# superlinear-ai/raglite

Measured on AMD Instinct MI355X. Metric: queries/sec, MaxSim 32x1M d=1024 exact top-100, higher is better.
Workload: dtype f32 in / f32 scores: candidate chunks found with the fp16 hi halves of corpus and queries (1 x v_mfma_f32_16x16x32_f16 per multiply, f32 accumulate, rigorous error bound), their scores by v_mfma_f32_16x16x4_f32 (exact f32 products); full-precision fallback: 3 x v_mfma_f32_16x16x32_f16 on hi+lo pairs

## Files before the change

raglite_amd/csrc/api.hip:

```cpp
#include <cmath>
#include <cstdlib>
#include <cstring>
#include <limits>
#include <memory>
#include <mutex>
#include <utility>
#include <vector>

#include "handles.h"

namespace rl {

static thread_local std::string g_last_error;
void set_error(const std::string& msg) { g_last_error = msg; }
int fail(int code, const std::string& msg) {
    g_last_error = msg;
    return code;
}

namespace {

int scan_mode(int metric) {
    switch (metric) {
        case RL_COSINE: return SCAN_COSINE;
// ... 106 lines not shown
bool image_fits(const rl_index* idx, const rl::Pool& pool, size_t need) {
    if (pool.cap >= need) return true;
    size_t free_b = 0, total_b = 0;
    if (hipMemGetInfo(&free_b, &total_b) != hipSuccess) { (void)hipGetLastError(); return true; }
    return free_b + pool.cap >= need + image_headroom(idx);
}
int64_t image_cap_rows(const rl_index* idx) { return std::max<int64_t>(idx->n_rows, idx->owns_E() ? idx->cap_rows : idx->n_rows); }

int refresh_ends(rl_index* idx, hipStream_t s) {
    if (idx->ends_rows == idx->n_rows && idx->ends.p) return RL_OK;
    RL_TRY(idx->ends.reserve(rl::chunk_ends_words(image_cap_rows(idx)) * sizeof(uint32_t)));
    RL_TRY(rl::launch_chunk_ends(idx->row_to_chunk, idx->n_rows, idx->ends.as<uint32_t>(), s));
    idx->ends_rows = idx->n_rows;
    return RL_OK;
}

int fold_row_norms(rl_index* idx, int64_t from, hipStream_t s) {
    rl::NormStats& ns = idx->norm_stats;
    RL_TRY(idx->d_norms.reserve(16));
    float w[4] = {ns.max_row_norm, ns.max_lo_norm, ns.max_lo_ratio, ns.min_row_norm};
    RL_HIP(hipMemcpyAsync(idx->d_norms, w, sizeof(w), hipMemcpyHostToDevice, s));
    const size_t at = (size_t)from * idx->dim;
    RL_TRY(idx->E16 ? rl::launch_max_row_norm16(idx->E16 + at, idx->n_rows - from, idx->dim, idx->d_norms, s)
                    : rl::launch_max_row_norm(idx->E + at, idx->n_rows - from, idx->dim, idx->split_scale, idx->d_norms, s));
    RL_HIP(hipMemcpyAsync(w, idx->d_norms, sizeof(w), hipMemcpyDeviceToHost, s));
    RL_HIP(hipStreamSynchronize(s));
    ns.max_row_norm = w[0];
    ns.max_lo_norm = w[1];
    ns.max_lo_ratio = w[2];
    ns.min_row_norm = w[3];
// ... 24 lines not shown
bool image_wanted(const rl_index* idx, uint32_t bit) {
    const int32_t d = idx->dim;
    if (!(image_need(idx) & bit) || idx->n_rows <= 0) return false;
    if (bit == IMG_PLANES) return idx->opt.on(RL_OPT_KEEP_IMAGE) && (idx->E16 || idx->E) && image_scale(idx) > 0.f && d % 32 == 0 && d >= 32;
    const bool hi = idx->opt.on(RL_OPT_KEEP_HI) && !idx->E16 && idx->E && idx->split_scale > 0.f && big_corpus(idx);
    if (bit == IMG_HI_IMAGE) return hi && hi_dim_ok(d);
    return hi && idx->opt.on(RL_OPT_KEEP_HI_PLANE) && stream16_dim_ok(d) &&
           (idx->metric == RL_COSINE || idx->metric == RL_DOT || idx->metric == RL_L2);
}

int refresh_image(rl_index* idx, uint32_t bit, hipStream_t s) {
    rl::Image& im = image_record(idx, bit);
    const bool tiled = bit != IMG_HI_PLANE;
    const int64_t n = idx->n_rows;
    const int32_t d = idx->dim;
    if (bit == IMG_PLANES) idx->ends_rows = -1;
    if (!image_wanted(idx, bit)) {
        im.drop();
        return RL_OK;
    }
    const float scale = image_scale(idx);
    const int64_t cap = image_cap_rows(idx);
    const size_t need = tiled ? rl::planes_bytes(cap, d, bit == IMG_HI_IMAGE || idx->E16) : (size_t)cap * d * sizeof(uint16_t);
    int64_t first = im.scale == scale ? (tiled ? im.rows & ~int64_t(15) : im.rows) : 0;
    if (im.buf.cap < need) first = 0;
    if (!image_fits(idx, im.buf, need) || im.buf.reserve(need) != RL_OK) {
        (void)hipGetLastError();
        idx->no_room |= bit;
        im.drop();
        return RL_OK;
    }
// ... 1449 lines not shown
    return (size_t)n * k * 3 + (size_t)n * 3 + 16 + (size_t)n * 2048 * 2 + 2 + 2 * pivot_scratch_words(std::min<int32_t>(n, 2));
}
int hi_batch_approx(rl_index* idx, const float* d_q, int32_t nq, int32_t n_queries, int32_t n_gemm, int32_t k, float* sc, int64_t ld, HiBatch& hb,
                    hipStream_t s, bool flag_zeroed = false) {
    hb.one_product = idx->opt.v[RL_OPT_HI_PRODUCTS] == 1;
    hb.exact_kth = idx->opt.on(RL_OPT_EXACT_KTH_THRESHOLD);
    RL_TRY(idx->hibuf.reserve(hi_batch_words(n_gemm, k) * 4));
    hi_batch_layout(idx, n_gemm, k, hb);
    const int32_t cap = hb.cap;
    hb.m_abs = idx->norm_stats.max_lo_norm + sum_eps(idx->dim) * idx->norm_stats.max_row_norm;
    hb.q_unscale = reinterpret_cast<const float*>(idx->qplanes.as<char>() + (size_t)n_queries * idx->dim * 128);
    hb.qsum = hb.q_unscale + 2 * (size_t)n_queries;
    if (!flag_zeroed) RL_HIP(hipMemsetAsync(hb.flag, 0, 16 * sizeof(uint32_t), s));
    (void)cap;
    const bool pp = hb.one_product && idx->dim >= 256 && idx->opt.on(RL_OPT_PP_PASS);
    if (pp)
        RL_TRY(launch_maxsim_pp(approx_image(idx), idx->n_rows, idx->dim, idx->qplanes.p, n_queries, 0, n_gemm, nq, idx->row_to_chunk,
                                idx->offsets, idx->ends.as<uint32_t>(), sc, ld, idx->n_cu, s, approx_scale(idx), nullptr,
                                (int)idx->opt.v[RL_OPT_PP_SCHEDULE], (int)idx->opt.v[RL_OPT_PP_XCD_PASSES]));
    for (int32_t b = 0; !pp && b < n_gemm; b += GEMM_PASS_QUERIES) {
        const int32_t n_q = std::min<int32_t>(GEMM_PASS_QUERIES, n_gemm - b);
        RL_TRY(launch_maxsim_gemm(approx_image(idx), idx->n_rows, idx->dim, idx->qplanes.p, n_queries, b, n_q, nq, idx->row_to_chunk,
                                  idx->offsets, idx->ends.as<uint32_t>(), sc + (int64_t)b * ld, ld, idx->n_cu, s, approx_scale(idx), true,
                                  nullptr, hb.one_product));
    }
    RL_TRY(mask_chunk_scores(idx, sc, n_gemm, ld, hb.filter, s));
    int st_pv = RL_ERR_UNSUPPORTED;
    if (n_gemm < 16 && idx->n_chunks > (int64_t)262144 && idx->opt.on(RL_OPT_HI_PIVOT))
        st_pv = launch_topk_pivot(sc, n_gemm, idx->n_chunks, ld, k, idx->ws, hb.ts, hb.ti, s);
    if (st_pv != RL_OK && st_pv != RL_ERR_UNSUPPORTED) return st_pv;
    if (st_pv == RL_ERR_UNSUPPORTED) RL_TRY(launch_topk(sc, n_gemm, idx->n_chunks, ld, k, idx->ws, hb.ts, hb.ti, s));
    return RL_OK;
}
int hi_batch_fallback(rl_index* idx, const float* d_q, int32_t nq, int32_t n_queries, int32_t n_gemm, int32_t k, float* sc, int64_t ld,
// ... 327 lines not shown
    if (idx->has_empty_chunk || idx->n_chunks == 0)
        return fail(RL_ERR_UNSUPPORTED, "rl_maxsim_approx_scores: the approximate pass needs an index without empty chunks");
    RL_TRY(demand_images(idx, approx_image_bit(idx), s));
    if (!approx_image_valid(idx) || nq > 32 || (kernel == 0 && idx->dim < 256))
        return fail(RL_ERR_UNSUPPORTED, "rl_maxsim_approx_scores: this index keeps no HI image (or nq > 32 / dim < 256)");
    Staging st(mem, s);
    const float* d_q; float* d_o; float* d_b = nullptr;
    const size_t q_elems = (size_t)nq * idx->dim;
    const int64_t ld = idx->n_chunks;
    RL_TRY(st.in(query_vecs, (size_t)n_queries * q_elems, &d_q));
    RL_TRY(st.out(out_scores, (size_t)n_queries * ld, &d_o));
    RL_TRY(st.out(out_bound, (size_t)n_queries, &d_b));
    RL_TRY(idx->qplanes.reserve(query_planes_bytes(idx->dim, n_queries)));
    RL_TRY(launch_query_planes(d_q, idx->dim, nq, (int64_t)q_elems, n_queries, idx->qplanes.p, s));
    const int32_t per = kernel == 0 ? n_queries : GEMM_PASS_QUERIES;
    for (int32_t b = 0; b < n_queries; b += per) {
        const int32_t n_q = std::min<int32_t>(per, n_queries - b);
        if (kernel == 0)
            RL_TRY(launch_maxsim_pp(approx_image(idx), idx->n_rows, idx->dim, idx->qplanes.p, n_queries, b, n_q, nq, idx->row_to_chunk, idx->offsets,
                                    idx->ends.as<uint32_t>(), d_o + (int64_t)b * ld, ld, idx->n_cu, s, approx_scale(idx), nullptr,
                                    (int)idx->opt.v[RL_OPT_PP_SCHEDULE], (int)idx->opt.v[RL_OPT_PP_XCD_PASSES]));
        else
            RL_TRY(launch_maxsim_gemm(approx_image(idx), idx->n_rows, idx->dim, idx->qplanes.p, n_queries, b, n_q, nq, idx->row_to_chunk, idx->offsets,
                                      idx->ends.as<uint32_t>(), d_o + (int64_t)b * ld, ld, idx->n_cu, s, approx_scale(idx), true, nullptr, true));
    }
    if (d_b) {
        const float m_abs = idx->norm_stats.max_lo_norm + sum_eps(idx->dim) * idx->norm_stats.max_row_norm;
        const float* q_unscale = reinterpret_cast<const float*>(idx->qplanes.as<char>() + (size_t)n_queries * idx->dim * 128);
        RL_TRY(idx->hibuf.reserve((size_t)n_queries * 4 * sizeof(float) + 64));
        float* top = idx->hibuf.as<float>();
        float* thr = top + n_queries;
        uint32_t* cnt = reinterpret_cast<uint32_t*>(thr + n_queries);
        uint32_t* flag = cnt + n_queries;
        RL_HIP(hipMemsetAsync(top, 0, (size_t)n_queries * sizeof(float), s));
        RL_HIP(hipMemsetAsync(flag, 0, 16 * sizeof(uint32_t), s));
// ... 195 lines not shown
    RL_HIP(hipEventCreate(&e0));
    RL_HIP(hipEventCreate(&e1));
    int st = RL_OK;
    if (kind == 2) {
        st = pairs_prepare(idx, q_dev, nq / 2, (int64_t)(nq / 2) * idx->dim, 2, s);
        if (st != RL_OK) { (void)hipEventDestroy(e0); (void)hipEventDestroy(e1); return st == RL_ERR_UNSUPPORTED ? fail(st, "rl_time_kernel: the pair kernel does not apply to this index / shape") : st; }
    }
    if (kind == 3 || kind == 5 || kind == 6) {
        st = gemm_prepare(idx, q_dev, nq / GEMM_PASS_QUERIES, (int64_t)(nq / GEMM_PASS_QUERIES) * idx->dim, GEMM_PASS_QUERIES, s, true);
        if (st == RL_OK && !image_valid(idx)) st = RL_ERR_UNSUPPORTED;
        if (st != RL_OK) { (void)hipEventDestroy(e0); (void)hipEventDestroy(e1); return st == RL_ERR_UNSUPPORTED ? fail(st, "rl_time_kernel: the eight-query kernel does not apply to this index / shape") : st; }
    }
    if (kind == 7) {
        st = pp_vec >= 1 && pp_vec * pp_n == nq ? gemm_prepare(idx, q_dev, pp_vec, (int64_t)pp_vec * idx->dim, pp_n, s) : RL_ERR_UNSUPPORTED;
        if (st == RL_OK && !(approx_image_valid(idx) && idx->dim >= 256)) st = RL_ERR_UNSUPPORTED;
        if (st != RL_OK) { (void)hipEventDestroy(e0); (void)hipEventDestroy(e1); return st == RL_ERR_UNSUPPORTED ? fail(st, "rl_time_kernel: the sixteen-query kernel does not apply to this index / shape") : st; }
    }
    if (kind == 4 || kind == 10) {
        st = demand_images(idx, IMG_HI_PLANE, s);
        if (st != RL_OK) { (void)hipEventDestroy(e0); (void)hipEventDestroy(e1); return st; }
    }
    RL_HIP(hipEventRecord(e0, s));
    for (int i = 0; i < iters && st == RL_OK; ++i) {
        if (kind == 7) st = launch_maxsim_pp(approx_image(idx), idx->n_rows, idx->dim, idx->qplanes.p, pp_n, 0, pp_n,
                                             pp_vec, idx->row_to_chunk, idx->offsets, idx->ends.as<uint32_t>(), idx->scores.as<float>(), ldc,
                                             idx->n_cu, s, approx_scale(idx), nullptr, (int)idx->opt.v[RL_OPT_PP_SCHEDULE], (int)idx->opt.v[RL_OPT_PP_XCD_PASSES]);
        else if (kind == 3) st = gemm_pass(idx, nq / GEMM_PASS_QUERIES, GEMM_PASS_QUERIES, 0, GEMM_PASS_QUERIES, idx->scores.as<float>(), ldc, s);
        else if (kind == 8) {
            const auto& r = idx->replay;
            if (hipMemsetAsync(r.cnt, 0, (size_t)r.B * sizeof(uint32_t), s) != hipSuccess) st = RL_ERR_HIP;
            else if (r.pp && r.round1_tiles > 0) {
                CandArgs ca1 = r.ca;
                ca1.tau = r.thr1;
                st = launch_pp_rows_pass(idx->hi_image.buf.p, idx->n_rows, idx->dim, r.B, r.qs, idx->norm, r.mode, &ca1, idx->pp_work.p, r.log_cap, idx->n_cu, s,
                                         idx->split_scale, 0, r.round1_tiles, false, r.row_test);
                if (st == RL_OK)
                    st = launch_pp_rows_pass(idx->hi_image.buf.p, idx->n_rows, idx->dim, r.B, r.qs, idx->norm, r.mode, &r.ca, idx->pp_work.p, r.log_cap, idx->n_cu, s,
                                             idx->split_scale, r.round1_tiles, -1, true, r.row_test);
            }
            else if (r.pp) st = launch_pp_rows_pass(idx->hi_image.buf.p, idx->n_rows, idx->dim, r.B, r.qs, idx->norm, r.mode, &r.ca, idx->pp_work.p, r.log_cap,
// ... 39 lines not shown
```

raglite_amd/csrc/common.h:

```cpp
#pragma once
#include <hip/hip_runtime.h>
#include <stdint.h>

#include <algorithm>
#include <cstdlib>
#include <string>

#include "raglite_hip.h"

namespace rl {

void set_error(const std::string& msg);
int fail(int code, const std::string& msg);

#define RL_HIP(expr)                                                                         \
    do {                                                                                     \
        hipError_t _e = (expr);                                                              \
        if (_e != hipSuccess)                                                                \
            return ::rl::fail(_e == hipErrorOutOfMemory ? RL_ERR_NOMEM : RL_ERR_HIP,         \
                              std::string(#expr) + ": " + hipGetErrorString(_e));            \
    } while (0)

#define RL_TRY(expr)              \
    do {                          \
// ... 382 lines not shown
                          float* out, int64_t out_stride, int n_cu, hipStream_t s, float split_scale);
size_t planes_bytes(int64_t rows, int32_t dim, bool half = false);
int launch_presplit_rows(const float* E, int64_t first_row, int64_t n_rows, int32_t dim, float scale, void* planes, hipStream_t s);
int launch_preformat_rows16(const uint16_t* E, int64_t first_row, int64_t n_rows, int32_t dim, void* planes, hipStream_t s);
int launch_presplit_hi_rows(const float* E, int64_t first_row, int64_t n_rows, int32_t dim, float scale, void* planes, hipStream_t s);
size_t chunk_ends_words(int64_t rows);
int launch_chunk_ends(const int32_t* row_to_chunk, int64_t n_rows, uint32_t* ends, hipStream_t s);
size_t query_planes_bytes(int32_t dim, int32_t n_queries);
int launch_query_planes(const float* Q, int32_t dim, int32_t nq, int64_t q_stride, int32_t n_queries, void* buf, hipStream_t s,
                        uint32_t* zero_words = nullptr, int n_zero = 0);
int launch_maxsim_gemm(const void* planes, int64_t n_rows, int32_t dim, const void* qbuf, int32_t n_queries, int32_t first,
                       int32_t n_q, int32_t nq, const int32_t* row_to_chunk, const int64_t* chunk_offsets, const uint32_t* ends_bits,
                       float* out, int64_t out_stride, int n_cu, hipStream_t s, float split_scale, bool half = false,
                       const uint32_t* run_if = nullptr, bool hi_only = false, bool all_passes = false);
constexpr int32_t PP_PASS_QUERIES = 16;
int launch_maxsim_pp(const void* image, int64_t n_rows, int32_t dim, const void* qbuf, int32_t n_queries, int32_t first, int32_t n_q,
                     int32_t nq, const int32_t* row_to_chunk, const int64_t* chunk_offsets, const uint32_t* ends_bits, float* out,
                     int64_t out_stride, int n_cu, hipStream_t s, float split_scale, const uint32_t* run_if, int schedule, int xcd_passes);
constexpr int32_t MFMA_RATE_ITERS = 1000;
int launch_mfma_f16_rate(float* out, int n_cu, int32_t iters, hipStream_t s, double* flops);
size_t score_planes_scratch_floats(int32_t nb, int32_t dim);
int launch_score_planes(const void* planes, int64_t n_rows, int32_t dim, const float* Q, int32_t nb, float* scores, int64_t ld,
                        const float* row_norm, const float* row_sumsq, float* scratch, int mode, int n_cu, hipStream_t s, float split_scale,
                        bool half = false);
struct CandArgs { const float* tau; int32_t tau_stride; float* scores; int32_t* ids; uint32_t* cnt; uint32_t* overflow; int32_t cap; };
int launch_score_planes_queries(const float* Q, int32_t nb, int32_t dim, float* scratch, int mode, hipStream_t s, uint32_t* zero_word = nullptr);
size_t pp_rows_scratch_bytes(int64_t n_rows, int32_t nb, int n_cu, int32_t expected_per_query, int32_t* log_cap_out);
int launch_pp_rows_pass(const void* image, int64_t n_rows, int32_t dim, int32_t nb, float* scratch, const float* row_norm, int mode,
                        const CandArgs* cand, void* work, int32_t log_cap, int n_cu, hipStream_t s, float split_scale, int64_t tile_begin = 0,
                        int64_t tile_count = -1, bool norms_ready = false,
                        bool row_norm_test = false);
int launch_pp_rows_sample(const void* image, int64_t n_rows, int32_t dim, int32_t nb, float* scratch, const float* row_norm, int mode, float* S,
// ... 33 lines not shown
```

raglite_amd/csrc/handles.h:

```cpp
#pragma once
#include <limits>
#include <memory>
#include <mutex>
#include <vector>

#include "device_mem.h"

namespace rl {

inline int filters_mem(int mem) { return (mem & RL_MEM_FILTERS_DEVICE) ? RL_MEM_DEVICE : mem; }
inline int args_mem(int mem) { return mem & ~RL_MEM_FILTERS_DEVICE; }

constexpr size_t SCORE_BATCH_BYTES = size_t(8) << 30;

struct Options {
    int64_t v[RL_OPT_PP_XCD_PASSES + 1];
    Options() {
        for (auto& x : v) x = 0;
        v[RL_OPT_HI_SEARCH] = v[RL_OPT_HI_MAXSIM] = v[RL_OPT_HI_PRODUCTS] = v[RL_OPT_PP_PASS] = v[RL_OPT_FUSED_TOPK] = v[RL_OPT_FUSED_HI] = 1;
        v[RL_OPT_FUSED_PP] = v[RL_OPT_GEMM_PASS] = v[RL_OPT_QUERY_PAIRS] = v[RL_OPT_PLANES_GEMM] = v[RL_OPT_KEEP_IMAGE] = v[RL_OPT_KEEP_HI] = 1;
        v[RL_OPT_EXACT_KTH_THRESHOLD] = v[RL_OPT_FUSED_TWO_ROUNDS] = v[RL_OPT_KEEP_HI_PLANE] = v[RL_OPT_F16_EXACT] = v[RL_OPT_LAZY_IMAGES] = v[RL_OPT_FUSED_PP_SAMPLE] = v[RL_OPT_LIST_SELECT] = v[RL_OPT_HI_FEW] = 1;
        v[RL_OPT_TOPK_BLOCK] = v[RL_OPT_PAIRS_PACKED] = 2;
        v[RL_OPT_HI_PIVOT] = 1;
        v[RL_OPT_PP_SCHEDULE] = 1;
// ... 97 lines not shown
    rl::Pool ends, qplanes;
    rl::Pool q32;
    rl::Pool cand;
    rl::Pool fused;
    rl::Pool pp_work;
    rl::Pool rankbuf;
    rl::Pool hybrid;
    rl::Pool rerank;
    rl::Image hiplane;
    rl::Pool hibuf;
    rl::Image hi_image;
    rl::NormStats norm_stats;
    rl::DevArray<uint32_t> d_norms;
    rl::LastStream last_stream;
    int64_t ends_rows = -1;
    int32_t rank_B = 0;
    int32_t mb_B = 0, mb_nq = 0, mb_k = 0;
    uint64_t scratch_epoch = 0, mb_epoch = 0;
    rl::Pool rank_q;
    struct FilterRecord { int kind = 0; int32_t n = 0, cap = 0; const uint32_t* cnt = nullptr; const uint32_t* flag = nullptr; } filt;
    rl::Options opt;
    uint32_t demanded = 0;
    uint32_t no_room = 0;
    uint64_t no_room_retry_epoch = 0;
    std::unique_ptr<uint32_t, hipError_t (*)(void*)> h_fell_back{nullptr, hipHostFree};
    uint32_t* d_fell_back = nullptr;
    struct FusedReplay {
        bool valid = false, pp = false, row_test = false; int32_t B = 0, log_cap = 0; int mode = 0; float* qs = nullptr; rl::CandArgs ca{}; uint32_t* cnt = nullptr;
        const float* thr1 = nullptr; int64_t round1_tiles = 0;
        const void* pools[3] = {nullptr, nullptr, nullptr};
// ... 42 lines not shown
```

raglite_amd/csrc/maxsim_pp.hip:

```cpp
#include <cstdio>
#include <cstdlib>
#include <utility>

#include "common.h"
#include "pp_schedule.h"

namespace rl {

typedef float f32x4 __attribute__((ext_vector_type(4)));
typedef _Float16 h16x8 __attribute__((ext_vector_type(8)));

namespace {
constexpr int PP_RT = 128;
constexpr int PP_NBLK = PP_RT / 16;
constexpr int PP_QPP = 16;
constexpr int PP_DC = 8;
constexpr int PP_LC = 6;
constexpr int PP_CSLOT = PP_NBLK * 1024;
constexpr int PP_STAGE = 1536;
constexpr int PP_LDS = PP_DC * PP_CSLOT + 16 * PP_STAGE * 4;

__device__ __forceinline__ int64_t pp_uniform_i64(int64_t v) {
    const uint32_t lo = __builtin_amdgcn_readfirstlane((uint32_t)(uint64_t)v);
    const uint32_t hi = __builtin_amdgcn_readfirstlane((uint32_t)((uint64_t)v >> 32));
// ... 43 lines not shown
    const float* q_unscale;
    const float* q_sumsq;
    const float* row_norm;
    const float* blk_minmax;
    int32_t B, QT, metric;
    float* cand_scores; int32_t* cand_ids; uint32_t* cand_cnt; uint32_t* overflow; int32_t cap;
    uint2* log; int32_t log_cap;
    int32_t tile_begin, tile_count;
    float* S; int64_t ld_s; int32_t stride;
    int32_t xcd_passes, dma_hint;
};

template <int DBG, int MODE, bool ROWNORM>
__global__ __launch_bounds__(512, 2) void maxsim_pp_kernel(const char* __restrict__ planes, int64_t n_rows, int32_t nslab,
                                                           const char* __restrict__ qfrag, const float* __restrict__ qmeta, int32_t n_q,
                                                           const int32_t* __restrict__ row_to_chunk, const int64_t* __restrict__ chunk_offsets,
                                                           const uint32_t* __restrict__ ends_bits, float* __restrict__ out, int64_t out_stride,
                                                           float inv_e_scale, const uint32_t* __restrict__ run_if, PpRows rs) {
    constexpr bool ROWS = MODE == 2, SCORES = MODE == 1, GROUPS = ROWS || SCORES;
    __shared__ __attribute__((aligned(16))) char smem[PP_LDS];
    if (run_if && __builtin_amdgcn_readfirstlane((int)*run_if) == 0) return;
    const int lane = threadIdx.x & 63;
    const int wv = wave_id();
    int64_t G = gridDim.x, b = blockIdx.x;
    int qt = (int)blockIdx.y;
    if constexpr (!GROUPS) {
        const int32_t passes = (n_q + PP_QPP - 1) / PP_QPP;
        const PpSlot m = gridDim.y > 1 ? pp_schedule((int32_t)blockIdx.x, (int32_t)blockIdx.y, (int32_t)gridDim.x, (int32_t)gridDim.y, passes)
                                       : pp_schedule_affine((int32_t)blockIdx.x, (int32_t)gridDim.x, passes, rs.xcd_passes);
        G = __builtin_amdgcn_readfirstlane(m.ranges);
        b = __builtin_amdgcn_readfirstlane(m.range);
        qt = __builtin_amdgcn_readfirstlane(m.pass);
    }
    auto boundary = [&](int64_t t) -> int64_t {
        if (t <= 0) return 0;
        if (t >= n_rows) return n_rows;
        const int32_t c = row_to_chunk[t];
        const int64_t c0 = chunk_offsets[c], c1 = chunk_offsets[c + 1];
        return c0 == t ? t : c1;
    };
    int32_t r_lo = 0, r_hi = 0, nt_rows = 0;
    if constexpr (!GROUPS) {
        r_lo = (int32_t)pp_uniform_i64(boundary((n_rows * b) / G));
        r_hi = (int32_t)pp_uniform_i64((b + 1 == G) ? n_rows : boundary((n_rows * (b + 1)) / G));
        if (r_hi <= r_lo) return;
    } else {
        const int64_t Tr = rs.tile_count;
        const int64_t t0 = (Tr * b) / G, t1 = (Tr * (b + 1)) / G;
        nt_rows = (int32_t)(t1 - t0);
        if (nt_rows <= 0) return;
        r_lo = (int32_t)((rs.tile_begin + t0) * PP_RT);
        r_hi = (int32_t)n_rows;
    }
    const int32_t org = r_lo & ~15;
    const int nt = GROUPS ? nt_rows : (r_hi - org + PP_RT - 1) / PP_RT;
    auto tile_blk = [&](int t) __attribute__((always_inline)) -> int32_t {
        if constexpr (SCORES) {
            const int32_t o = (org >> 7) + t;
            return ((o >> 1) * 2 * rs.stride + (o & 1)) * PP_NBLK;
// ... 60 lines not shown
    auto mfma_group = [&](f32x4 (&q)[4], auto A_) __attribute__((always_inline)) {
        constexpr int A = decltype(A_)::value;
        if constexpr (!(DBG & 2)) {
            acc[0][0][A] = __builtin_amdgcn_mfma_f32_16x16x32_f16(pp_h(ef[A]), pp_h(q[0]), acc[0][0][A], 0, 0, 0);
            acc[0][1][A] = __builtin_amdgcn_mfma_f32_16x16x32_f16(pp_h(ef[A]), pp_h(q[1]), acc[0][1][A], 0, 0, 0);
            acc[1][0][A] = __builtin_amdgcn_mfma_f32_16x16x32_f16(pp_h(ef[A]), pp_h(q[2]), acc[1][0][A], 0, 0, 0);
            acc[1][1][A] = __builtin_amdgcn_mfma_f32_16x16x32_f16(pp_h(ef[A]), pp_h(q[3]), acc[1][1][A], 0, 0, 0);
        }
    };

    const int fG = lane >> 4, fb = (lane >> 2) & 3, ft = lane & 3;
    const int my_row = (ft >> 1) + 2 * (fb & 1) + 4 * (fb >> 1) + 8 * (fG & 1);
    const uint32_t my_bit = 1u << my_row, my_below = my_bit - 1u;
    float run = -INFINITY;
    uint32_t prev_last_end = 1;
    int32_t ord_run = GROUPS ? 0 : __builtin_amdgcn_readfirstlane(row_to_chunk[org]);
    const int e_q = fG >> 1;
    const bool e_has = !GROUPS && (e_q == 0 ? has0 : has1) && (ft & 1) == 0;
    const float e_unscale = e_has ? qmeta[2 * (q_base + 2 * wv + e_q)] * inv_e_scale : 0.f;
    [[maybe_unused]] float* const o_buf = reinterpret_cast<float*>(smem + PP_DC * PP_CSLOT) + (2 * wv + e_q) * PP_STAGE;
    [[maybe_unused]] const int32_t ord_lo = !GROUPS ? __builtin_amdgcn_readfirstlane(row_to_chunk[r_lo]) : 0;
    [[maybe_unused]] int32_t own_cnt = 0, own_flushed = 0;
    [[maybe_unused]] auto flush_out = [&]() __attribute__((always_inline)) {
        if constexpr (!GROUPS) {
            const int n = own_cnt - own_flushed;
            asm volatile("s_waitcnt lgkmcnt(0)" ::: "memory");
            const float* const b0 = reinterpret_cast<const float*>(smem + PP_DC * PP_CSLOT) + (2 * wv) * PP_STAGE;
            float* const g0 = out + (int64_t)(q_base + 2 * wv) * out_stride + ord_lo + own_flushed;
            if (has0)
                for (int i = lane; i < n; i += 64) g0[i] = b0[i];
            if (has1)
                for (int i = lane; i < n; i += 64) g0[out_stride + i] = b0[PP_STAGE + i];
            own_flushed = own_cnt;
            asm volatile("s_waitcnt vmcnt(0)" ::: "memory");
        }
    };
// ... 400 lines not shown
    flush_out();
    if constexpr (DBG & 128) {
        if (n_q > 1000000) {
            f32x4 t = (f32x4){0.f, 0.f, 0.f, 0.f};
#pragma unroll
            for (int q = 0; q < 2; ++q)
#pragma unroll
                for (int qb = 0; qb < 2; ++qb)
#pragma unroll
                    for (int a = 0; a < PP_NBLK; ++a) t += acc[q][qb][a];
            out[lane] = (t[0] + t[1]) + (t[2] + t[3]);
        }
    }
}

int launch_maxsim_pp(const void* image, int64_t n_rows, int32_t dim, const void* qbuf, int32_t n_queries, int32_t first, int32_t n_q,
                     int32_t nq, const int32_t* row_to_chunk, const int64_t* chunk_offsets, const uint32_t* ends_bits, float* out,
                     int64_t out_stride, int n_cu, hipStream_t s, float split_scale, const uint32_t* run_if, int schedule, int xcd_passes) {
    if (nq < 1 || nq > 32 || n_q < 1 || n_q > PP_QPP * 4096 || n_rows < 1 || first < 0 || first + n_q > n_queries) return RL_ERR_UNSUPPORTED;
    if (dim % 32 || dim < 256 || !(split_scale > 0.f) || !image || !ends_bits) return RL_ERR_UNSUPPORTED;
    const int32_t nslab = dim / 32;
    const char* qfrag = static_cast<const char*>(qbuf) + (size_t)first * nslab * 4096;
    const float* qmeta = reinterpret_cast<const float*>(static_cast<const char*>(qbuf) + (size_t)n_queries * dim * 128) + 2 * (size_t)first;
    const int64_t tiles = (n_rows + PP_RT - 1) / PP_RT;
    const int64_t gx = std::max<int64_t>(1, std::min<int64_t>(n_cu > 0 ? n_cu : 256, tiles)), passes = (n_q + PP_QPP - 1) / PP_QPP;
    const dim3 grid = schedule == 1 ? dim3((unsigned)(gx * passes)) : dim3((unsigned)gx, (unsigned)passes), blk(512);
    PpRows rs{};
    rs.xcd_passes = schedule == 1 ? xcd_passes : 8;
#define RL_PP_LAUNCH(DBG_)                                                                                                                 \
    hipLaunchKernelGGL((maxsim_pp_kernel<DBG_, 0, false>), grid, blk, 0, s, static_cast<const char*>(image), n_rows, nslab, qfrag, qmeta, n_q, row_to_chunk, \
                       chunk_offsets, ends_bits, out, out_stride, 1.0f / split_scale, run_if, rs)
#ifdef RAGLITE_EXPERIMENTS
    const int force_hint = std::getenv("RAGLITE_PP_HINT") ? std::atoi(std::getenv("RAGLITE_PP_HINT")) : -1;
    if (force_hint >= PP_HINT_NONE && force_hint <= PP_HINT_SC1) rs.dma_hint = force_hint;
    static const int dbg = std::getenv("RAGLITE_PP_DBG") ? std::atoi(std::getenv("RAGLITE_PP_DBG")) : 0;
    if (dbg == 2) RL_PP_LAUNCH(2);
    else if (dbg == 128) RL_PP_LAUNCH(128);
    else if (dbg == 136) RL_PP_LAUNCH(136);
    else if (dbg == 144) RL_PP_LAUNCH(144);
    else if (dbg == 160) RL_PP_LAUNCH(160);
    else if (dbg == 184) RL_PP_LAUNCH(184);
    else RL_PP_LAUNCH(0);
#else
    RL_PP_LAUNCH(0);
#endif
#undef RL_PP_LAUNCH
// ... 24 lines not shown
    float* frag = scratch;
    float* unscale = frag + (size_t)groups * 32 * dim;
    float* anylo = unscale + nb;
    float* qss = anylo + groups;
    const int64_t grid_cu = n_cu > 0 ? n_cu : 256;
    const int64_t T256 = (n_rows + 255) / 256, Tv = (T256 + stride - 1) / stride;
    if (Tv * 256 != ld_s) return RL_ERR_INVALID;
    PpRows rs{};
    rs.tile_begin = 0;
    rs.tile_count = (int32_t)(2 * Tv);
    rs.q_unscale = unscale; rs.q_sumsq = qss; rs.row_norm = row_norm; rs.B = nb; rs.QT = (groups + PP_QPP - 1) / PP_QPP; rs.metric = mode;
    rs.S = S; rs.ld_s = ld_s; rs.stride = stride;
    if (rs.QT > grid_cu) return RL_ERR_UNSUPPORTED;
    const int64_t gx = std::max<int64_t>(1, std::min<int64_t>(grid_cu / rs.QT, 2 * Tv));
    hipLaunchKernelGGL((maxsim_pp_kernel<0, 1, false>), dim3((unsigned)gx, (unsigned)rs.QT), dim3(512), 0, s, static_cast<const char*>(image), n_rows,
                       nslab, reinterpret_cast<const char*>(frag), nullptr, groups, nullptr, nullptr, nullptr, nullptr, (int64_t)0,
                       1.0f / split_scale, nullptr, rs);
    RL_HIP(hipGetLastError());
    return RL_OK;
}

size_t pp_rows_scratch_bytes(int64_t n_rows, int32_t nb, int n_cu, int32_t expected_per_query, int32_t* log_cap_out) {
    const int64_t grid = n_cu > 0 ? n_cu : 256;
    int64_t cap = ((int64_t)expected_per_query * nb * 4) / (grid * 8) + 1;
    cap = std::max<int64_t>(4096, (cap + 1023) & ~int64_t(1023));
    cap = std::min<int64_t>(cap, int64_t(1) << 19);
    if (log_cap_out) *log_cap_out = (int32_t)cap;
    const size_t blocks = (size_t)((n_rows + 15) / 16);
    return (size_t)grid * 8 * (size_t)cap * sizeof(uint2) + blocks * 2 * sizeof(float) + 256;
}

// ... 20 lines not shown
    rs.tau = cand->tau; rs.q_unscale = unscale; rs.q_sumsq = qss; rs.row_norm = row_norm; rs.B = nb; rs.QT = (groups + PP_QPP - 1) / PP_QPP;
    rs.metric = mode; rs.cand_scores = cand->scores; rs.cand_ids = cand->ids; rs.cand_cnt = cand->cnt; rs.overflow = cand->overflow; rs.cap = cand->cap;
    rs.log = static_cast<uint2*>(work);
    rs.log_cap = log_cap;
    if (rs.QT > grid_cu || Tr_all + 2 >= (int64_t(1) << 19)) return RL_ERR_UNSUPPORTED;
    float* blk_mm = reinterpret_cast<float*>(static_cast<char*>(work) + (size_t)grid_cu * 8 * (size_t)log_cap * sizeof(uint2));
    rs.blk_minmax = blk_mm;
    if (mode == SCAN_COSINE && !norms_ready) {
        const int64_t n_blocks = (n_rows + 15) / 16;
        hipLaunchKernelGGL(block_norm_minmax_kernel, dim3((unsigned)((n_blocks + 255) / 256)), dim3(256), 0, s, row_norm, n_rows, n_blocks, blk_mm);
    }
    const int64_t gx = std::max<int64_t>(1, std::min<int64_t>(grid_cu / rs.QT, Tr));
    const dim3 grid((unsigned)gx, (unsigned)rs.QT), blk(512);
#define RL_PP_ROWS(DBG_, RN_)                                                                                                             \
    hipLaunchKernelGGL((maxsim_pp_kernel<DBG_, 2, RN_>), grid, blk, 0, s, static_cast<const char*>(image), n_rows, nslab, reinterpret_cast<const char*>(frag), \
                       nullptr, groups, nullptr, nullptr, nullptr, nullptr, (int64_t)0, 1.0f / split_scale, nullptr, rs)
#ifdef RAGLITE_EXPERIMENTS
    static const int dbg = std::getenv("RAGLITE_PP_ROWS_DBG") ? std::atoi(std::getenv("RAGLITE_PP_ROWS_DBG")) : 0;
    if (dbg == 128) RL_PP_ROWS(128, false);
    else if (row_norm_test) RL_PP_ROWS(0, true);
    else RL_PP_ROWS(0, false);
#else
    if (row_norm_test) RL_PP_ROWS(0, true);
    else RL_PP_ROWS(0, false);
#endif
#undef RL_PP_ROWS
    RL_HIP(hipGetLastError());
    return RL_OK;
}

__global__ __launch_bounds__(512, 2) void mfma_f16_rate_kernel(float* __restrict__ out, int32_t iters) {
// ... 47 lines not shown
```

Before: 18440.

## Precompute chunk-aligned row ranges for the sixteen-query kernel with a tile-balanced plan

```diff
diff --git a/raglite_amd/csrc/api.hip b/raglite_amd/csrc/api.hip
--- a/raglite_amd/csrc/api.hip
+++ b/raglite_amd/csrc/api.hip
@@ -8,6 +8,7 @@
 #include <vector>
 
 #include "handles.h"
+#include "pp_plan.h"
 
 namespace rl {
 
@@ -144,6 +145,15 @@
     idx->ends_rows = idx->n_rows;
     return RL_OK;
 }
+int refresh_pp_plan(rl_index* idx, int32_t ranges, hipStream_t s) {
+    if (idx->pp_plan_rows == idx->n_rows && idx->pp_plan_ranges == ranges && idx->pp_plan.p) return RL_OK;
+    idx->pp_plan_rows = -1;
+    RL_TRY(idx->pp_plan.reserve(rl::pp_plan_bytes(ranges)));
+    RL_TRY(rl::launch_pp_plan(idx->row_to_chunk, idx->offsets, idx->n_rows, ranges, idx->pp_plan.as<rl::PpRange>(), s));
+    idx->pp_plan_rows = idx->n_rows;
+    idx->pp_plan_ranges = ranges;
+    return RL_OK;
+}
 
 int fold_row_norms(rl_index* idx, int64_t from, hipStream_t s) {
     rl::NormStats& ns = idx->norm_stats;
@@ -198,7 +208,7 @@
     const bool tiled = bit != IMG_HI_PLANE;
     const int64_t n = idx->n_rows;
     const int32_t d = idx->dim;
-    if (bit == IMG_PLANES) idx->ends_rows = -1;
+    if (bit == IMG_PLANES) idx->ends_rows = idx->pp_plan_rows = -1;
     if (!image_wanted(idx, bit)) {
         im.drop();
         return RL_OK;
@@ -1678,10 +1688,12 @@
     if (!flag_zeroed) RL_HIP(hipMemsetAsync(hb.flag, 0, 16 * sizeof(uint32_t), s));
     (void)cap;
     const bool pp = hb.one_product && idx->dim >= 256 && idx->opt.on(RL_OPT_PP_PASS);
-    if (pp)
-        RL_TRY(launch_maxsim_pp(approx_image(idx), idx->n_rows, idx->dim, idx->qplanes.p, n_queries, 0, n_gemm, nq, idx->row_to_chunk,
-                                idx->offsets, idx->ends.as<uint32_t>(), sc, ld, idx->n_cu, s, approx_scale(idx), nullptr,
+    if (pp) {
+        RL_TRY(refresh_pp_plan(idx, pp_ranges(idx->n_rows, idx->n_cu), s));
+        RL_TRY(launch_maxsim_pp(approx_image(idx), idx->n_rows, idx->dim, idx->qplanes.p, n_queries, 0, n_gemm, nq, idx->pp_plan.as<PpRange>(),
+                                idx->pp_plan_ranges, idx->ends.as<uint32_t>(), sc, ld, idx->n_cu, s, approx_scale(idx), nullptr,
                                 (int)idx->opt.v[RL_OPT_PP_SCHEDULE], (int)idx->opt.v[RL_OPT_PP_XCD_PASSES]));
+    }
     for (int32_t b = 0; !pp && b < n_gemm; b += GEMM_PASS_QUERIES) {
         const int32_t n_q = std::min<int32_t>(GEMM_PASS_QUERIES, n_gemm - b);
         RL_TRY(launch_maxsim_gemm(approx_image(idx), idx->n_rows, idx->dim, idx->qplanes.p, n_queries, b, n_q, nq, idx->row_to_chunk,
@@ -2039,11 +2051,12 @@
     RL_TRY(idx->qplanes.reserve(query_planes_bytes(idx->dim, n_queries)));
     RL_TRY(launch_query_planes(d_q, idx->dim, nq, (int64_t)q_elems, n_queries, idx->qplanes.p, s));
     const int32_t per = kernel == 0 ? n_queries : GEMM_PASS_QUERIES;
+    if (kernel == 0) RL_TRY(refresh_pp_plan(idx, pp_ranges(idx->n_rows, idx->n_cu), s));
     for (int32_t b = 0; b < n_queries; b += per) {
         const int32_t n_q = std::min<int32_t>(per, n_queries - b);
         if (kernel == 0)
-            RL_TRY(launch_maxsim_pp(approx_image(idx), idx->n_rows, idx->dim, idx->qplanes.p, n_queries, b, n_q, nq, idx->row_to_chunk, idx->offsets,
-                                    idx->ends.as<uint32_t>(), d_o + (int64_t)b * ld, ld, idx->n_cu, s, approx_scale(idx), nullptr,
+            RL_TRY(launch_maxsim_pp(approx_image(idx), idx->n_rows, idx->dim, idx->qplanes.p, n_queries, b, n_q, nq, idx->pp_plan.as<PpRange>(),
+                                    idx->pp_plan_ranges, idx->ends.as<uint32_t>(), d_o + (int64_t)b * ld, ld, idx->n_cu, s, approx_scale(idx), nullptr,
                                     (int)idx->opt.v[RL_OPT_PP_SCHEDULE], (int)idx->opt.v[RL_OPT_PP_XCD_PASSES]));
         else
             RL_TRY(launch_maxsim_gemm(approx_image(idx), idx->n_rows, idx->dim, idx->qplanes.p, n_queries, b, n_q, nq, idx->row_to_chunk, idx->offsets,
@@ -2269,6 +2282,7 @@
     if (kind == 7) {
         st = pp_vec >= 1 && pp_vec * pp_n == nq ? gemm_prepare(idx, q_dev, pp_vec, (int64_t)pp_vec * idx->dim, pp_n, s) : RL_ERR_UNSUPPORTED;
         if (st == RL_OK && !(approx_image_valid(idx) && idx->dim >= 256)) st = RL_ERR_UNSUPPORTED;
+        if (st == RL_OK) st = refresh_pp_plan(idx, pp_ranges(idx->n_rows, idx->n_cu), s);
         if (st != RL_OK) { (void)hipEventDestroy(e0); (void)hipEventDestroy(e1); return st == RL_ERR_UNSUPPORTED ? fail(st, "rl_time_kernel: the sixteen-query kernel does not apply to this index / shape") : st; }
     }
     if (kind == 4 || kind == 10) {
@@ -2278,7 +2292,7 @@
     RL_HIP(hipEventRecord(e0, s));
     for (int i = 0; i < iters && st == RL_OK; ++i) {
         if (kind == 7) st = launch_maxsim_pp(approx_image(idx), idx->n_rows, idx->dim, idx->qplanes.p, pp_n, 0, pp_n,
-                                             pp_vec, idx->row_to_chunk, idx->offsets, idx->ends.as<uint32_t>(), idx->scores.as<float>(), ldc,
+                                             pp_vec, idx->pp_plan.as<PpRange>(), idx->pp_plan_ranges, idx->ends.as<uint32_t>(), idx->scores.as<float>(), ldc,
                                              idx->n_cu, s, approx_scale(idx), nullptr, (int)idx->opt.v[RL_OPT_PP_SCHEDULE], (int)idx->opt.v[RL_OPT_PP_XCD_PASSES]);
         else if (kind == 3) st = gemm_pass(idx, nq / GEMM_PASS_QUERIES, GEMM_PASS_QUERIES, 0, GEMM_PASS_QUERIES, idx->scores.as<float>(), ldc, s);
         else if (kind == 8) {
diff --git a/raglite_amd/csrc/common.h b/raglite_amd/csrc/common.h
--- a/raglite_amd/csrc/common.h
+++ b/raglite_amd/csrc/common.h
@@ -420,8 +420,12 @@
                        float* out, int64_t out_stride, int n_cu, hipStream_t s, float split_scale, bool half = false,
                        const uint32_t* run_if = nullptr, bool hi_only = false, bool all_passes = false);
 constexpr int32_t PP_PASS_QUERIES = 16;
+struct PpRange;
+int32_t pp_ranges(int64_t n_rows, int n_cu);
+size_t pp_plan_bytes(int32_t ranges);
+int launch_pp_plan(const int32_t* row_to_chunk, const int64_t* chunk_offsets, int64_t n_rows, int32_t ranges, PpRange* plan, hipStream_t s);
 int launch_maxsim_pp(const void* image, int64_t n_rows, int32_t dim, const void* qbuf, int32_t n_queries, int32_t first, int32_t n_q,
-                     int32_t nq, const int32_t* row_to_chunk, const int64_t* chunk_offsets, const uint32_t* ends_bits, float* out,
+                     int32_t nq, const PpRange* plan, int32_t plan_ranges, const uint32_t* ends_bits, float* out,
                      int64_t out_stride, int n_cu, hipStream_t s, float split_scale, const uint32_t* run_if, int schedule, int xcd_passes);
 constexpr int32_t MFMA_RATE_ITERS = 1000;
 int launch_mfma_f16_rate(float* out, int n_cu, int32_t iters, hipStream_t s, double* flops);
diff --git a/raglite_amd/csrc/handles.h b/raglite_amd/csrc/handles.h
--- a/raglite_amd/csrc/handles.h
+++ b/raglite_amd/csrc/handles.h
@@ -135,6 +135,9 @@
     rl::DevArray<uint32_t> d_norms;
     rl::LastStream last_stream;
     int64_t ends_rows = -1;
+    rl::Pool pp_plan;
+    int64_t pp_plan_rows = -1;
+    int32_t pp_plan_ranges = 0;
     int32_t rank_B = 0;
     int32_t mb_B = 0, mb_nq = 0, mb_k = 0;
     uint64_t scratch_epoch = 0, mb_epoch = 0;
diff --git a/raglite_amd/csrc/maxsim_pp.hip b/raglite_amd/csrc/maxsim_pp.hip
--- a/raglite_amd/csrc/maxsim_pp.hip
+++ b/raglite_amd/csrc/maxsim_pp.hip
@@ -3,6 +3,7 @@
 #include <utility>
 
 #include "common.h"
+#include "pp_plan.h"
 #include "pp_schedule.h"
 
 namespace rl {
@@ -81,35 +82,28 @@
 template <int DBG, int MODE, bool ROWNORM>
 __global__ __launch_bounds__(512, 2) void maxsim_pp_kernel(const char* __restrict__ planes, int64_t n_rows, int32_t nslab,
                                                            const char* __restrict__ qfrag, const float* __restrict__ qmeta, int32_t n_q,
-                                                           const int32_t* __restrict__ row_to_chunk, const int64_t* __restrict__ chunk_offsets,
-                                                           const uint32_t* __restrict__ ends_bits, float* __restrict__ out, int64_t out_stride,
+                                                           const PpRange* __restrict__ plan, const uint32_t* __restrict__ ends_bits,
+                                                           float* __restrict__ out, int64_t out_stride,
                                                            float inv_e_scale, const uint32_t* __restrict__ run_if, PpRows rs) {
     constexpr bool ROWS = MODE == 2, SCORES = MODE == 1, GROUPS = ROWS || SCORES;
     __shared__ __attribute__((aligned(16))) char smem[PP_LDS];
     if (run_if && __builtin_amdgcn_readfirstlane((int)*run_if) == 0) return;
     const int lane = threadIdx.x & 63;
     const int wv = wave_id();
-    int64_t G = gridDim.x, b = blockIdx.x;
+    const int64_t G = gridDim.x, b = blockIdx.x;
     int qt = (int)blockIdx.y;
+    int32_t r_lo = 0, r_hi = 0, nt_rows = 0;
+    [[maybe_unused]] int32_t plan_ord_org = 0, plan_ord_lo = 0;
     if constexpr (!GROUPS) {
         const int32_t passes = (n_q + PP_QPP - 1) / PP_QPP;
         const PpSlot m = gridDim.y > 1 ? pp_schedule((int32_t)blockIdx.x, (int32_t)blockIdx.y, (int32_t)gridDim.x, (int32_t)gridDim.y, passes)
                                        : pp_schedule_affine((int32_t)blockIdx.x, (int32_t)gridDim.x, passes, rs.xcd_passes);
-        G = __builtin_amdgcn_readfirstlane(m.ranges);
-        b = __builtin_amdgcn_readfirstlane(m.range);
+        const PpRange pr = plan[__builtin_amdgcn_readfirstlane(m.range)];
         qt = __builtin_amdgcn_readfirstlane(m.pass);
-    }
-    auto boundary = [&](int64_t t) -> int64_t {
-        if (t <= 0) return 0;
-        if (t >= n_rows) return n_rows;
-        const int32_t c = row_to_chunk[t];
-        const int64_t c0 = chunk_offsets[c], c1 = chunk_offsets[c + 1];
-        return c0 == t ? t : c1;
-    };
-    int32_t r_lo = 0, r_hi = 0, nt_rows = 0;
-    if constexpr (!GROUPS) {
-        r_lo = (int32_t)pp_uniform_i64(boundary((n_rows * b) / G));
-        r_hi = (int32_t)pp_uniform_i64((b + 1 == G) ? n_rows : boundary((n_rows * (b + 1)) / G));
+        r_lo = __builtin_amdgcn_readfirstlane(pr.r_lo);
+        r_hi = __builtin_amdgcn_readfirstlane(pr.r_hi);
+        plan_ord_org = __builtin_amdgcn_readfirstlane(pr.ord_org);
+        plan_ord_lo = __builtin_amdgcn_readfirstlane(pr.ord_lo);
         if (r_hi <= r_lo) return;
     } else {
         const int64_t Tr = rs.tile_count;
@@ -200,12 +194,12 @@
     const uint32_t my_bit = 1u << my_row, my_below = my_bit - 1u;
     float run = -INFINITY;
     uint32_t prev_last_end = 1;
-    int32_t ord_run = GROUPS ? 0 : __builtin_amdgcn_readfirstlane(row_to_chunk[org]);
+    int32_t ord_run = plan_ord_org;
     const int e_q = fG >> 1;
     const bool e_has = !GROUPS && (e_q == 0 ? has0 : has1) && (ft & 1) == 0;
     const float e_unscale = e_has ? qmeta[2 * (q_base + 2 * wv + e_q)] * inv_e_scale : 0.f;
     [[maybe_unused]] float* const o_buf = reinterpret_cast<float*>(smem + PP_DC * PP_CSLOT) + (2 * wv + e_q) * PP_STAGE;
-    [[maybe_unused]] const int32_t ord_lo = !GROUPS ? __builtin_amdgcn_readfirstlane(row_to_chunk[r_lo]) : 0;
+    [[maybe_unused]] const int32_t ord_lo = plan_ord_lo;
     [[maybe_unused]] int32_t own_cnt = 0, own_flushed = 0;
     [[maybe_unused]] auto flush_out = [&]() __attribute__((always_inline)) {
         if constexpr (!GROUPS) {
@@ -636,22 +630,50 @@
     }
 }
 
+int32_t pp_ranges(int64_t n_rows, int n_cu) {
+    const int64_t tiles = (n_rows + PP_RT - 1) / PP_RT;
+    return (int32_t)std::max<int64_t>(1, std::min<int64_t>(n_cu > 0 ? n_cu : 256, tiles));
+}
+size_t pp_plan_bytes(int32_t ranges) { return (size_t)ranges * sizeof(PpRange); }
+
+__global__ __launch_bounds__(64) void pp_plan_kernel(const int32_t* __restrict__ row_to_chunk, const int64_t* __restrict__ chunk_offsets,
+                                                     int64_t n_rows, int32_t G, PpRange* __restrict__ plan) {
+    if (blockIdx.x != 0 || threadIdx.x != 0) return;
+    auto chunk_of = [&](int64_t t) {
+        const int32_t c = row_to_chunk[t];
+        return PpChunk{chunk_offsets[c], chunk_offsets[c + 1]};
+    };
+    int64_t lo = 0;
+    for (int32_t b = 0; b < G; ++b) {
+        const int64_t hi = pp_plan_next(n_rows, G, b, lo, chunk_of);
+        const bool some = hi > lo;
+        plan[b] = PpRange{(int32_t)lo, (int32_t)hi, some ? row_to_chunk[lo & ~int64_t(15)] : 0, some ? row_to_chunk[lo] : 0};
+        lo = hi;
+    }
+}
+int launch_pp_plan(const int32_t* row_to_chunk, const int64_t* chunk_offsets, int64_t n_rows, int32_t ranges, PpRange* plan, hipStream_t s) {
+    if (!row_to_chunk || !chunk_offsets || !plan || n_rows < 1 || n_rows > INT32_MAX || ranges < 1) return RL_ERR_UNSUPPORTED;
+    hipLaunchKernelGGL(pp_plan_kernel, dim3(1), dim3(64), 0, s, row_to_chunk, chunk_offsets, n_rows, ranges, plan);
+    RL_HIP(hipGetLastError());
+    return RL_OK;
+}
+
 int launch_maxsim_pp(const void* image, int64_t n_rows, int32_t dim, const void* qbuf, int32_t n_queries, int32_t first, int32_t n_q,
-                     int32_t nq, const int32_t* row_to_chunk, const int64_t* chunk_offsets, const uint32_t* ends_bits, float* out,
+                     int32_t nq, const PpRange* plan, int32_t plan_ranges, const uint32_t* ends_bits, float* out,
                      int64_t out_stride, int n_cu, hipStream_t s, float split_scale, const uint32_t* run_if, int schedule, int xcd_passes) {
     if (nq < 1 || nq > 32 || n_q < 1 || n_q > PP_QPP * 4096 || n_rows < 1 || first < 0 || first + n_q > n_queries) return RL_ERR_UNSUPPORTED;
     if (dim % 32 || dim < 256 || !(split_scale > 0.f) || !image || !ends_bits) return RL_ERR_UNSUPPORTED;
     const int32_t nslab = dim / 32;
     const char* qfrag = static_cast<const char*>(qbuf) + (size_t)first * nslab * 4096;
     const float* qmeta = reinterpret_cast<const float*>(static_cast<const char*>(qbuf) + (size_t)n_queries * dim * 128) + 2 * (size_t)first;
-    const int64_t tiles = (n_rows + PP_RT - 1) / PP_RT;
-    const int64_t gx = std::max<int64_t>(1, std::min<int64_t>(n_cu > 0 ? n_cu : 256, tiles)), passes = (n_q + PP_QPP - 1) / PP_QPP;
+    const int64_t gx = pp_ranges(n_rows, n_cu), passes = (n_q + PP_QPP - 1) / PP_QPP;
+    if (!plan || plan_ranges != gx) return RL_ERR_INVALID;
     const dim3 grid = schedule == 1 ? dim3((unsigned)(gx * passes)) : dim3((unsigned)gx, (unsigned)passes), blk(512);
     PpRows rs{};
     rs.xcd_passes = schedule == 1 ? xcd_passes : 8;
 #define RL_PP_LAUNCH(DBG_)                                                                                                                 \
-    hipLaunchKernelGGL((maxsim_pp_kernel<DBG_, 0, false>), grid, blk, 0, s, static_cast<const char*>(image), n_rows, nslab, qfrag, qmeta, n_q, row_to_chunk, \
-                       chunk_offsets, ends_bits, out, out_stride, 1.0f / split_scale, run_if, rs)
+    hipLaunchKernelGGL((maxsim_pp_kernel<DBG_, 0, false>), grid, blk, 0, s, static_cast<const char*>(image), n_rows, nslab, qfrag, qmeta, n_q, plan, \
+                       ends_bits, out, out_stride, 1.0f / split_scale, run_if, rs)
 #ifdef RAGLITE_EXPERIMENTS
     const int force_hint = std::getenv("RAGLITE_PP_HINT") ? std::atoi(std::getenv("RAGLITE_PP_HINT")) : -1;
     if (force_hint >= PP_HINT_NONE && force_hint <= PP_HINT_SC1) rs.dma_hint = force_hint;
@@ -706,7 +728,7 @@
     if (rs.QT > grid_cu) return RL_ERR_UNSUPPORTED;
     const int64_t gx = std::max<int64_t>(1, std::min<int64_t>(grid_cu / rs.QT, 2 * Tv));
     hipLaunchKernelGGL((maxsim_pp_kernel<0, 1, false>), dim3((unsigned)gx, (unsigned)rs.QT), dim3(512), 0, s, static_cast<const char*>(image), n_rows,
-                       nslab, reinterpret_cast<const char*>(frag), nullptr, groups, nullptr, nullptr, nullptr, nullptr, (int64_t)0,
+                       nslab, reinterpret_cast<const char*>(frag), nullptr, groups, nullptr, nullptr, nullptr, (int64_t)0,
                        1.0f / split_scale, nullptr, rs);
     RL_HIP(hipGetLastError());
     return RL_OK;
@@ -757,7 +779,7 @@
     const dim3 grid((unsigned)gx, (unsigned)rs.QT), blk(512);
 #define RL_PP_ROWS(DBG_, RN_)                                                                                                             \
     hipLaunchKernelGGL((maxsim_pp_kernel<DBG_, 2, RN_>), grid, blk, 0, s, static_cast<const char*>(image), n_rows, nslab, reinterpret_cast<const char*>(frag), \
-                       nullptr, groups, nullptr, nullptr, nullptr, nullptr, (int64_t)0, 1.0f / split_scale, nullptr, rs)
+                       nullptr, groups, nullptr, nullptr, nullptr, (int64_t)0, 1.0f / split_scale, nullptr, rs)
 #ifdef RAGLITE_EXPERIMENTS
     static const int dbg = std::getenv("RAGLITE_PP_ROWS_DBG") ? std::atoi(std::getenv("RAGLITE_PP_ROWS_DBG")) : 0;
     if (dbg == 128) RL_PP_ROWS(128, false);
diff --git a/raglite_amd/csrc/pp_plan.h b/raglite_amd/csrc/pp_plan.h
--- /dev/null
+++ b/raglite_amd/csrc/pp_plan.h
@@ -0,0 +1,44 @@
+#pragma once
+#include <stdint.h>
+
+#if defined(__HIPCC__) || defined(__CUDACC__)
+#define RL_PP_PLAN_HD __host__ __device__
+#else
+#define RL_PP_PLAN_HD
+#endif
+
+namespace rl {
+
+constexpr int32_t PP_PLAN_TILE = 128;
+
+struct PpChunk {
+    int64_t start, end;
+};
+
+struct alignas(16) PpRange {
+    int32_t r_lo, r_hi;
+    int32_t ord_org;
+    int32_t ord_lo;
+};
+
+template <class ChunkOf>
+RL_PP_PLAN_HD inline int64_t pp_plan_next(int64_t n_rows, int32_t G, int32_t b, int64_t B_b, ChunkOf&& chunk_of) {
+    if (b + 1 >= G || B_b >= n_rows) return n_rows;
+    const int64_t org = B_b & ~int64_t(15), share = (int64_t)PP_PLAN_TILE * (G - b);
+    const int64_t m = (n_rows - org + share - 1) / share, budget = org + PP_PLAN_TILE * m;
+    if (budget >= n_rows) return n_rows;
+    const int64_t at = chunk_of(budget).start;
+    return at > B_b ? at : chunk_of(B_b).end;
+}
+
+template <class ChunkOf>
+RL_PP_PLAN_HD inline void pp_plan(int64_t n_rows, int32_t G, int64_t* B, ChunkOf&& chunk_of) {
+    B[0] = 0;
+    for (int32_t b = 0; b < G; ++b) B[b + 1] = pp_plan_next(n_rows, G, b, B[b], chunk_of);
+}
+
+RL_PP_PLAN_HD inline int64_t pp_plan_tiles(int64_t lo, int64_t hi) {
+    return hi > lo ? (hi - (lo & ~int64_t(15)) + PP_PLAN_TILE - 1) / PP_PLAN_TILE : 0;
+}
+
+}
```

New measurement: 18610, median of 6. No clear change (+0.9%).
